# thekingofkings/embedding

Hardware: AMD Instinct MI355X
Metric: SGNS training edges/sec (higher is better)
Workload: dtype f32

## Files before the change

embedding_amd/_native.py:

```python
import ctypes as C
import os

_HERE = os.path.dirname(os.path.abspath(__file__))
LIB_PATH = os.path.join(_HERE, "libdge.so")

DGE_OK, DGE_ERR_ARG, DGE_ERR_RANGE, DGE_ERR_TOPK, DGE_ERR_CAP, DGE_ERR_STATE, DGE_ERR_DEVICE, DGE_ERR_IO = range(8)


class DgeError(RuntimeError):
    def __init__(self, code, msg):
        super().__init__("libdge error %d: %s" % (code, msg))
        self.code = code


class TrainConfig(C.Structure):
    _fields_ = [
        ("dim", C.c_int32), ("window", C.c_int32), ("negative", C.c_int32), ("min_count", C.c_int32),
        ("epochs", C.c_int32), ("workers", C.c_int32), ("alpha", C.c_float), ("min_alpha", C.c_float),
        ("seed", C.c_uint64), ("table_size", C.c_int64), ("n_vertices", C.c_int32), ("update_policy", C.c_int32),
        ("use_hs", C.c_int32), ("reserved", C.c_int32),
    ]


class TrainStats(C.Structure):
# ... 103 lines not shown
    "dge_regions_centroids": (_int, [_vp, _vp, _i64, _P(_i64)]),
    "dge_graph_add_spatial": (_int, [_vp, _vp, _i32, _dbl, _vp, _P(SpatialInfo)]),
    "dge_graph_add_spatial_points": (_int, [_vp, _vp, _vp, _i64, _i32, _dbl, _vp, _P(SpatialInfo)]),
    "dge_trips_parse_texts": (_int, [_int, _vp, _vp, _i32, _P(TripTextOptions), _vp, _vp, _vp, _vp, _i64, _P(_i64), _P(TripTextInfo)]),
    "dge_flows_add_trip_texts": (_int, [_vp, _vp, _vp, _i32, _P(TripTextOptions), _P(TripTextInfo)]),
    "dge_flows_add_trip_files": (_int, [_vp, _vp, _i32, _P(TripTextOptions), _P(TripTextInfo)]),
    "dge_sample_walks": (_int, [_vp, _i64, _i32, _i64, _int, _i64, _vp, _P(_i64)]),
    "dge_sample_walks_device": (_int, [_vp, _i64, _i32, _i64, _int, _i64, _P(_vp), _P(_i64)]),
    "dge_sample_walks_into": (_int, [_vp, _vp, _i64, _i64, _i64, _i64]),
    "dge_walks_from_host": (_int, [_int, _vp, _i64, _i32, _P(_vp)]),
    "dge_names_create": (_int, [_P(_vp)]),
    "dge_names_add": (_int, [_vp, _vp, _i64]),
    "dge_names_count": (_int, [_vp, _P(_i64)]),
    "dge_names_cstrs": (_int, [_vp, _P(_vp)]),
    "dge_names_free": (None, [_vp]),
    "dge_walks_from_seq_text": (_int, [_int, _vp, _i64, _vp, _int, _P(_vp), _P(SeqInfo)]),
    "dge_walks_from_seq_files": (_int, [_int, _vp, _i32, _vp, _int, _P(_vp), _P(SeqInfo)]),
    "dge_walks_to_seq_text": (_int, [_vp, _i64, _i64, _vp, _int, _vp, _i64, _P(_i64), _P(SeqOutInfo)]),
    "dge_walks_write_seq": (_int, [_vp, _i64, _i64, _vp, _int, C.c_char_p, _int, _P(SeqOutInfo)]),
    "dge_walks_to_host": (_int, [_vp, _vp, _i64]),
    "dge_walks_info": (_int, [_vp, _P(_i64), _P(_i32), _P(_vp)]),
    "dge_walks_add_position_prefix": (_int, [_vp, _i32]),
    "dge_walks_free": (None, [_vp]),
    "dge_count_tokens": (_int, [_vp, _i64, _i64, _i32, _vp]),
    "dge_model_create": (_int, [_int, _P(TrainConfig), _vp, _P(_vp)]),
    "dge_model_set_stream": (_int, [_vp, _vp]),
    "dge_model_train": (_int, [_vp, _vp, _i64, _i64, _i64, _i32, _i64, _dbl, _i64]),
    "dge_train_sgns": (_int, [_int, _vp, _i64, _i32, _P(TrainConfig), _P(_vp)]),
    "dge_train_sgns_device": (_int, [_vp, _P(TrainConfig), _P(_vp)]),
    "dge_model_walk_and_train": (_int, [_vp, _vp, _vp, _i64, _i64, _i64, _i64, _i32, _i64, _dbl, _i64]),
    "dge_model_vectors": (_int, [_vp, _P(_vp), _P(_vp), _P(_i64), _P(_i32)]),
    "dge_model_syn1neg": (_int, [_vp, _P(_vp)]),
    "dge_model_syn1": (_int, [_vp, _P(_vp), _P(_i64)]),
    "dge_model_huffman": (_int, [_vp, _P(_vp), _P(_vp), _P(_vp)]),
    "dge_model_counts": (_int, [_vp, _P(_vp)]),
    "dge_model_table": (_int, [_vp, _P(_vp), _P(_i64)]),
    "dge_model_stats": (_int, [_vp, _P(TrainStats)]),
    "dge_model_row_rates": (_int, [_vp, _P(C.c_double), _P(C.c_double), _P(C.c_double), _P(C.c_double)]),
    "dge_model_table_placement": (_int, [_vp, _i32, _vp, _vp, _vp]),
    "dge_model_table_runs": (_int, [_vp, _vp, _vp]),
    "dge_model_tune_placement": (_int, [_vp, _vp, _i64, _i64, _i32, _vp, _vp, _vp]),
    "dge_model_placement_search": (_int, [_vp, _vp, _vp, _vp, _vp]),
    "dge_model_reset_stats": (_int, [_vp]),
    "dge_model_schedule": (_int, [_vp, _P(_i32), _P(_i64), _P(_i32)]),
    "dge_model_kernel": (_int, [_vp, C.c_char_p, _i32]),
    "dge_model_lock_stats": (_int, [_vp, _P(_i64), _P(_i64), _P(_i64)]),
    "dge_model_score_pairs": (_int, [_vp, _vp, _vp, _i64, _vp]),
    "dge_model_eval_links": (_int, [_vp, _vp, _i64, _i64, _i32, C.c_uint64, _P(EvalResult)]),
    "dge_model_eval_sgns": (_int, [_vp, _vp, _i64, _i64, C.c_uint64, _P(EvalResult)]),
    "dge_write_vec": (_int, [_vp, _vp, C.c_char_p, _int]),
    "dge_model_free": (None, [_vp]),
    "dge_model_set_partition": (_int, [_vp, _i32, _i32, _i32]),
    "dge_model_partition_floats": (_int, [_vp, _i32, _P(_i64)]),
    "dge_model_export_partition": (_int, [_vp, _int, _i32, _i32, _vp]),
    "dge_model_import_partition": (_int, [_vp, _int, _i32, _i32, _vp]),
    "dge_model_export_partition_async": (_int, [_vp, _int, _i32, _i32, _vp, _vp]),
    "dge_model_import_partition_async": (_int, [_vp, _int, _i32, _i32, _vp, _vp]),
    "dge_model_stream": (_int, [_vp, _P(_vp)]),
    "dge_host_sync_count": (_int, [_P(_i64)]),
    "dge_model_sync_size": (_int, [_vp, _P(_i64)]),
    "dge_model_snapshot": (_int, [_vp]),
    "dge_model_export_delta": (_int, [_vp, _vp]),
    "dge_model_import_delta": (_int, [_vp, _vp, C.c_float]),
    "dge_comm_unique_id": (_int, [_vp]),
    "dge_comm_create": (_int, [_P(_vp), _vp, _int, _int, _int]),
    "dge_comm_free": (None, [_vp]),
# ... 61 lines not shown
```

embedding_amd/csrc/sgns_io.hip:

```cpp
#include <string.h>

#include <algorithm>
#include <charconv>
#include <string>
#include <thread>
#include <vector>

#include "dge_internal.h"
#include "sgns_kernels.h"
#include "sgns_model.h"
#include "fmt_g9.h"

static int sync_tables_to_host(dge_model* m, bool want_syn0, bool want_syn1, bool want_hs = false) {
    DGE_HIP(hipSetDevice(m->device));
    DGE_HIP(hipStreamSynchronize(m->stream));
    size_t tab = (size_t)m->V * (size_t)m->stride;
    std::vector<float> tmp(tab ? tab : 1);
    for (int which = 0; which < 3; which++) {
        if ((which == 0 && !want_syn0) || (which == 1 && !want_syn1) || (which == 2 && !want_hs)) continue;
        const float* src = which == 0 ? m->d_syn0 : (which == 1 ? m->d_syn1neg : m->d_syn1);
        if (tab) DGE_HIP(hipMemcpy(tmp.data(), src, tab * sizeof(float), hipMemcpyDeviceToHost));
        std::vector<float>& dst = which == 0 ? m->h_syn0 : (which == 1 ? m->h_syn1neg : m->h_syn1);
        const int64_t rows = which == 2 ? std::max<int64_t>(m->V - 1, 0) : m->V;
        dst.resize((size_t)rows * (size_t)m->D + 1);
        for (int64_t r = 0; r < rows; r++) memcpy(dst.data() + r * m->D, tmp.data() + r * m->stride, (size_t)m->D * sizeof(float));
    }
    return DGE_OK;
}

extern "C" int dge_model_vectors(dge_model* m, const float** syn0, const int32_t** vocab_ids, int64_t* V, int32_t* dim) {
    if (!m) DGE_FAIL(DGE_ERR_ARG, "dge_model_vectors: null model");
    int rc = sync_tables_to_host(m, true, false);
    if (rc) return rc;
    if (syn0) *syn0 = m->h_syn0.data();
    if (vocab_ids) *vocab_ids = m->h_vocab_ids.data();
    if (V) *V = m->V;
    if (dim) *dim = m->D;
    return DGE_OK;
}
extern "C" int dge_model_syn1neg(dge_model* m, const float** syn1neg) {
    if (!m || !syn1neg) DGE_FAIL(DGE_ERR_ARG, "dge_model_syn1neg: null argument");
    int rc = sync_tables_to_host(m, false, true);
    if (rc) return rc;
    *syn1neg = m->h_syn1neg.data();
    return DGE_OK;
}
extern "C" int dge_model_syn1(dge_model* m, const float** syn1, int64_t* rows) {
    if (!m || !syn1) DGE_FAIL(DGE_ERR_ARG, "dge_model_syn1: null argument");
    if (!m->d_syn1) DGE_FAIL(DGE_ERR_STATE, "dge_model_syn1: the model was created without use_hs");
    int rc = sync_tables_to_host(m, false, false, true);
    if (rc) return rc;
    *syn1 = m->h_syn1.data();
    if (rows) *rows = std::max<int64_t>(m->V - 1, 0);
    return DGE_OK;
}
extern "C" int dge_model_huffman(dge_model* m, const int64_t** offsets, const int32_t** points, const uint64_t** codes) {
    if (!m) DGE_FAIL(DGE_ERR_ARG, "dge_model_huffman: null model");
    if (!m->d_syn1) DGE_FAIL(DGE_ERR_STATE, "dge_model_huffman: the model was created without use_hs");
    if (offsets) *offsets = m->h_hs_off.data();
    if (points) *points = m->h_hs_points.data();
    if (codes) *codes = m->h_hs_codes.data();
    return DGE_OK;
}
extern "C" int dge_model_counts(dge_model* m, const int64_t** counts) {
    if (!m || !counts) DGE_FAIL(DGE_ERR_ARG, "dge_model_counts: null argument");
    *counts = m->h_counts.data();
    return DGE_OK;
}
__global__ void k_table_unpack(const uint4* __restrict__ ctab, int64_t T, int32_t* __restrict__ table) {
    const int64_t a = (int64_t)blockIdx.x * blockDim.x + threadIdx.x;
    if (a < T) table[a] = neg_table_row(ctab, (uint64_t)a);
}
extern "C" int dge_model_table(dge_model* m, const int32_t** table, int64_t* table_size) {
    if (!m || !table) DGE_FAIL(DGE_ERR_ARG, "dge_model_table: null argument");
    DGE_HIP(hipSetDevice(m->device));
    m->h_table.resize((size_t)m->T);
    dge_tmp<int32_t> flat;
    int rc = flat.alloc((size_t)m->T);
    if (rc) return rc;
    DGE_HIP(hipStreamSynchronize(m->stream));
    hipLaunchKernelGGL(k_table_unpack, dim3(dge_grid_for(m->T, 256)), dim3(256), 0, m->stream, m->d_ctab, m->T, flat.p);
    DGE_HIP(hipStreamSynchronize(m->stream));
    DGE_HIP(hipMemcpy(m->h_table.data(), flat.p, (size_t)m->T * sizeof(int32_t), hipMemcpyDeviceToHost));
    *table = m->h_table.data();
    if (table_size) *table_size = m->T;
    return DGE_OK;
}

extern "C" int dge_write_vec(dge_model* m, const char* const* names, const char* path, int header) {
    if (!m || !path) DGE_FAIL(DGE_ERR_ARG, "dge_write_vec: null argument");
    int rc = sync_tables_to_host(m, true, false);
    if (rc) return rc;
    FILE* f = fopen(path, "w");
    if (!f) DGE_FAIL(DGE_ERR_IO, "dge_write_vec: cannot open %s", path);
    if (header) fprintf(f, "%lld %d\n", (long long)m->V, m->D);
    const int64_t V = m->V; const int D = m->D;
    const unsigned hw = std::thread::hardware_concurrency();
    const int n_thr = (int)std::max<int64_t>(1, std::min<int64_t>(std::min<unsigned>(hw ? hw : 1, 16u), V * (int64_t)D / 65536));
    const int64_t slab = 4096 * (int64_t)n_thr;
    std::vector<std::string> out[2] = {std::vector<std::string>((size_t)n_thr), std::vector<std::string>((size_t)n_thr)};
    bool ok = true;
    std::thread writer;
    int cur = 0;
    for (int64_t r0 = 0; r0 < V; r0 += slab, cur ^= 1) {
        const int64_t r1 = std::min(V, r0 + slab);
        std::vector<std::string>& ob = out[cur];
        auto work = [&, r0, r1](int t) {
            std::string& sbuf = ob[(size_t)t];
            const int64_t a = r0 + (r1 - r0) * t / n_thr, b = r0 + (r1 - r0) * (t + 1) / n_thr;
            size_t cap = 0;
            for (int64_t r = a; r < b; r++) { const int32_t id = m->h_vocab_ids[(size_t)r]; cap += (names && names[id] ? strlen(names[id]) : 12) + (size_t)D * 26 + 2; }
            sbuf.resize(cap);
            char* o = sbuf.data();
            for (int64_t r = a; r < b; r++) {
                const int32_t id = m->h_vocab_ids[(size_t)r];
                if (names && names[id]) { const size_t n = strlen(names[id]); memcpy(o, names[id], n); o += n; } else o = std::to_chars(o, o + 12, id).ptr;
                const float* v = m->h_syn0.data() + r * D;
                for (int j = 0; j < D; j++) {
                    *o++ = ' ';
                    char* e = dge_fmt_g9(v[j], o);
                    o = e ? e : std::to_chars(o, o + 25, (double)v[j], std::chars_format::general, 9).ptr;
                }
                *o++ = '\n';
            }
            sbuf.resize((size_t)(o - sbuf.data()));
        };
        if (n_thr == 1) work(0);
        else {
            std::vector<std::thread> th;
            for (int t = 0; t < n_thr; t++) th.emplace_back(work, t);
            for (auto& x : th) x.join();
        }
        if (writer.joinable()) writer.join();
        if (!ok) break;
        writer = std::thread([&ok, &ob, f, n_thr]() {
            for (int t = 0; t < n_thr && ok; t++) ok = ob[(size_t)t].empty() || fwrite(ob[(size_t)t].data(), 1, ob[(size_t)t].size(), f) == ob[(size_t)t].size();
        });
    }
    if (writer.joinable()) writer.join();
    if (fclose(f) != 0 || !ok) DGE_FAIL(DGE_ERR_IO, "dge_write_vec: write to %s failed", path);
    return DGE_OK;
}

__global__ void k_load_vectors(const int32_t* __restrict__ vocab_ids, int64_t V, int32_t D, int32_t stride, const float* __restrict__ rows, const uint8_t* __restrict__ present,
                               int64_t n_rows, float* __restrict__ syn0, unsigned long long* __restrict__ rows_set) {
    const int64_t i = (int64_t)blockIdx.x * blockDim.x + threadIdx.x;
    if (i >= V * D) return;
    const int64_t r = i / D; const int32_t j = (int32_t)(i - r * D);
    const int64_t id = vocab_ids[r];
    if (id < 0 || id >= n_rows || !present[id]) return;
    syn0[r * stride + j] = rows[id * D + j];
    if (j == 0) atomicAdd(rows_set, 1ull);
}

extern "C" int dge_model_load_vectors(dge_model* m, const dge_vectors* v, int64_t* rows_set) {
    if (!m || !v) DGE_FAIL(DGE_ERR_ARG, "dge_model_load_vectors: null argument");
    if (v->dim != m->D) DGE_FAIL(DGE_ERR_ARG, "dge_model_load_vectors: the vectors have dim %d, the model %d", v->dim, m->D);
    if (v->device != m->device) DGE_FAIL(DGE_ERR_ARG, "dge_model_load_vectors: the vectors are on device %d, the model on %d", v->device, m->device);
    if (m->part_n > 1) DGE_FAIL(DGE_ERR_STATE, "dge_model_load_vectors: a partition is set (n_parts = %d): the tables are in pieces — call dge_model_set_partition(m, 1, 0, 0) first", m->part_n);
    DGE_HIP(hipSetDevice(m->device));
    dge_tmp<unsigned long long> count;
    int rc = count.alloc(1);
    if (rc) return rc;
    DGE_HIP(hipMemsetAsync(count.p, 0, 8, m->stream));
    const int64_t n = m->V * (int64_t)m->D;
    if (n && v->rows) hipLaunchKernelGGL(k_load_vectors, dim3(dge_grid_for(n, 256)), dim3(256), 0, m->stream, m->d_vocab_ids, m->V, m->D, m->stride, v->d, v->d_present, v->rows, m->d_syn0,
                                         count.p);
    DGE_HIP(hipGetLastError());
    unsigned long long set = 0;
    DGE_HIP(hipMemcpyAsync(&set, count.p, 8, hipMemcpyDeviceToHost, m->stream));
    DGE_HIP(hipStreamSynchronize(m->stream));
    if (rows_set) *rows_set = (int64_t)set;
    return DGE_OK;
}
// ... 1 lines not shown
```

embedding_amd/csrc/sgns_model.h:

```cpp
#pragma once
#include <algorithm>
#include <atomic>
#include <string>
#include <vector>

#include "dge_internal.h"
#include "sgns_plan.h"

struct EventPair { hipEvent_t a, b; int kind; };

extern std::atomic<int64_t> g_dge_tuning[DGE_TUNE_COUNT];

struct dge_sorted_work;

struct dge_model {
    int device = 0;
    hipStream_t stream = nullptr;
    bool own_stream = false;
    dge_train_config cfg{};
    int64_t V = 0;
    int32_t D = 0, stride = 0, NV = 0;
    int64_t T = 0;
    ScheduleStats stats;
    BlockHeadMemo block_head_memo;
    int n_cus = 256;
    float *d_syn0 = nullptr, *d_syn1neg = nullptr, *d_snap = nullptr;
    int placed_seen[3] = {0, 0, 0}; double placed_best[3] = {0, 0, 0}, placed_worst[3] = {0, 0, 0};
    float* d_syn1 = nullptr;
    int64_t* d_hs_off = nullptr; int32_t* d_hs_points = nullptr; uint64_t* d_hs_codes = nullptr;
    std::vector<int64_t> h_hs_off; std::vector<int32_t> h_hs_points; std::vector<uint64_t> h_hs_codes;
    std::vector<float> h_syn1;

    int32_t* d_vocab_ids = nullptr;
    int64_t* d_counts = nullptr;
    int32_t* d_remap = nullptr;
    uint4* d_ctab = nullptr; int64_t ctab_blocks = 0;
    double* d_run_base = nullptr; uint32_t* d_run_row = nullptr; uint32_t* d_exc_slot = nullptr; int32_t* d_exc_row = nullptr;
    int32_t n_runs = 0, n_exc = 0;
    float* d_exp = nullptr;
    int64_t cap_rows = 0; int32_t cap_L = 0;
    int32_t* d_sen = nullptr; int64_t* d_len = nullptr; int64_t* d_wb = nullptr;
    void* d_scan_tmp = nullptr; size_t scan_tmp_bytes = 0;
    unsigned long long* d_counters = nullptr;
    int* d_locks = nullptr;
    std::vector<float> h_syn0, h_syn1neg;
    std::vector<int32_t> h_vocab_ids, h_table;
    std::vector<int64_t> h_counts;
    std::vector<EventPair> pending;
    double kernel_ms = 0, walk_ms = 0;
    int64_t launches = 0;
    TrainPlan last_plan; bool has_plan = false;
    int32_t search_runs = 0, search_moved = 0; double search_ms_before = 0, search_ms_after = 0;
    int32_t part_n = 1, part_ctx = 0, part_tgt = 0;
    const int32_t* seen_rows = nullptr; int64_t seen_n = 0; int32_t seen_L = 0; uint64_t seen_gen = 0;
    hipEvent_t ev_peer = nullptr;
    dge_sorted_work* sorted = nullptr;
};

struct TrainParams;
int dge_sorted_train(dge_model* m, const TrainParams& p);
void dge_sorted_release(dge_model* m);

#define DGE_LOCAL __attribute__((visibility("hidden")))
DGE_LOCAL int dge_table_alloc(float** out, size_t floats, int device, hipStream_t st, int* seen, double* rate_best, double* rate_worst);
DGE_LOCAL void dge_table_free(void* p);
DGE_LOCAL int dge_drain_events(dge_model* m);
static inline unsigned dge_grid_for(int64_t n, int block) { return (unsigned)((n + block - 1) / block); }
```

embedding_amd/engine.py:

```python
import ctypes as C
import os

import numpy as np

from ._native import DGE_ERR_CAP, DGE_SLOTS_AS_TRACTS, DGE_SLOTS_EVEN, EvalResult, FlowsInfo, LocateInfo, OdInfo, RegionsInfo, SeqInfo, SeqOutInfo, SpatialInfo, TrainConfig, TrainStats, TripTextInfo, TripTextOptions, VecInfo, check, lib


def _ptr(a):
    return a.ctypes.data_as(C.c_void_p) if a is not None else None


def _dev_ptr(t):
    if t is None:
        return None
    if isinstance(t, int):
        return C.c_void_p(t)
    return C.c_void_p(t.data_ptr())


class DeviceGraph:

    def __init__(self, device=0):
        h = C.c_void_p(0)
        check(lib.dge_graph_create(C.byref(h), int(device)))
# ... 571 lines not shown
    def fit(cls, walks, cfg, device=0):
        h = C.c_void_p(0)
        if isinstance(walks, WalkCorpus):
            check(lib.dge_train_sgns_device(walks._h, C.byref(cfg), C.byref(h)))
            device = walks.device
        else:
            walks = np.ascontiguousarray(walks, np.int32)
            n, L = walks.shape
            check(lib.dge_train_sgns(int(device), _ptr(walks), n, L, C.byref(cfg), C.byref(h)))
        return cls(h, int(device), cfg)

    def close(self):
        if getattr(self, "_h", None):
            lib.dge_model_free(self._h)
            self._h = None

    __del__ = close

    def set_stream(self, stream_ptr):
        check(lib.dge_model_set_stream(self._h, C.c_void_p(int(stream_ptr))))

    def train(self, corpus, row0=0, n_rows=None, walk_index_base=0, epoch=0, words_before=0, words_scale=1.0, total_walks=0):
        if n_rows is None:
            n_rows = corpus.shape[0] - row0
        check(lib.dge_model_train(self._h, corpus._h, int(row0), int(n_rows), int(walk_index_base), int(epoch),
                                  int(words_before), float(words_scale), int(total_walks)))

    def walk_and_train(self, graph, corpus, row0, n_rows, walk_seed, walk_index_base, epoch=0, words_before=0,
                       words_scale=1.0, total_walks=0):
        check(lib.dge_model_walk_and_train(self._h, graph._h, corpus._h, int(row0), int(n_rows), int(walk_seed),
                                           int(walk_index_base), int(epoch), int(words_before), float(words_scale),
                                           int(total_walks)))

    def vectors(self):
        p = C.c_void_p(0); ids = C.c_void_p(0); V = C.c_int64(0); D = C.c_int32(0)
        check(lib.dge_model_vectors(self._h, C.byref(p), C.byref(ids), C.byref(V), C.byref(D)))
        if V.value == 0:
            return np.zeros((0, D.value), np.float32), np.zeros(0, np.int32)
        syn0 = np.ctypeslib.as_array(C.cast(p, C.POINTER(C.c_float)), shape=(V.value * D.value,)).copy().reshape(V.value, D.value)
        vid = np.ctypeslib.as_array(C.cast(ids, C.POINTER(C.c_int32)), shape=(V.value,)).copy()
        return syn0, vid

    def syn1neg(self):
        syn0, _ = self.vectors()
        p = C.c_void_p(0)
        check(lib.dge_model_syn1neg(self._h, C.byref(p)))
        if syn0.size == 0:
            return np.zeros_like(syn0)
        return np.ctypeslib.as_array(C.cast(p, C.POINTER(C.c_float)), shape=(syn0.size,)).copy().reshape(syn0.shape)

    def syn1(self):
        p = C.c_void_p(0); rows = C.c_int64(0)
        check(lib.dge_model_syn1(self._h, C.byref(p), C.byref(rows)))
        n = rows.value * self.cfg.dim
        if n == 0:
            return np.zeros((0, self.cfg.dim), np.float32)
        return np.ctypeslib.as_array(C.cast(p, C.POINTER(C.c_float)), shape=(n,)).copy().reshape(rows.value, self.cfg.dim)

    def huffman(self):
        _, vid = self.vectors()
        V = len(vid)
        po, pp, pc = C.c_void_p(0), C.c_void_p(0), C.c_void_p(0)
        check(lib.dge_model_huffman(self._h, C.byref(po), C.byref(pp), C.byref(pc)))
        if V == 0:
            return np.zeros(1, np.int64), np.zeros(0, np.int32), np.zeros(0, np.uint64)
        off = np.ctypeslib.as_array(C.cast(po, C.POINTER(C.c_int64)), shape=(V + 1,)).copy()
        n = int(off[-1])
        pts = np.ctypeslib.as_array(C.cast(pp, C.POINTER(C.c_int32)), shape=(max(n, 1),)).copy()[:n]
        codes = np.ctypeslib.as_array(C.cast(pc, C.POINTER(C.c_uint64)), shape=(V,)).copy()
        return off, pts, codes

    def counts(self):
        _, vid = self.vectors()
        p = C.c_void_p(0)
        check(lib.dge_model_counts(self._h, C.byref(p)))
        if len(vid) == 0:
            return np.zeros(0, np.int64)
        return np.ctypeslib.as_array(C.cast(p, C.POINTER(C.c_int64)), shape=(len(vid),)).copy()

    def table(self):
        p = C.c_void_p(0); T = C.c_int64(0)
        check(lib.dge_model_table(self._h, C.byref(p), C.byref(T)))
        return np.ctypeslib.as_array(C.cast(p, C.POINTER(C.c_int32)), shape=(T.value,)).copy()

    def row_rates(self):
        v = [C.c_double(0) for _ in range(4)]
        check(lib.dge_model_row_rates(self._h, *[C.byref(x) for x in v])); return tuple(x.value for x in v)

    def table_runs(self):
        n, e = C.c_int32(0), C.c_int32(0)
# ... 95 lines not shown
    def import_partition(self, table, n_parts, part, d_buf):
        check(lib.dge_model_import_partition(self._h, int(table), int(n_parts), int(part), _dev_ptr(d_buf)))

    def export_partition_async(self, table, n_parts, part, d_buf, consumer_stream=0):
        check(lib.dge_model_export_partition_async(self._h, int(table), int(n_parts), int(part), _dev_ptr(d_buf), C.c_void_p(int(consumer_stream))))

    def import_partition_async(self, table, n_parts, part, d_buf, producer_stream=0):
        check(lib.dge_model_import_partition_async(self._h, int(table), int(n_parts), int(part), _dev_ptr(d_buf), C.c_void_p(int(producer_stream))))

    def stream(self):
        p = C.c_void_p(0); check(lib.dge_model_stream(self._h, C.byref(p))); return p.value or 0

    def sync_size(self):
        n = C.c_int64(0); check(lib.dge_model_sync_size(self._h, C.byref(n))); return n.value

    def snapshot(self):
        check(lib.dge_model_snapshot(self._h))

    def export_delta(self, d_buf):
        check(lib.dge_model_export_delta(self._h, _dev_ptr(d_buf)))

    def import_delta(self, d_buf, scale):
        check(lib.dge_model_import_delta(self._h, _dev_ptr(d_buf), float(scale)))


def host_sync_count():
    n = C.c_int64(0); check(lib.dge_host_sync_count(C.byref(n))); return n.value


def build_stamp():
    return dict(kv.split("=") for kv in lib.dge_build_stamp().decode().split())


TUNING_KNOBS = {"hot_rows": 0, "hs_drain": 1, "force_segments": 2, "segment_shift": 3, "sorted_chunk": 4, "sorted_walks": 5, "workers": 6, "static_walks": 7, "hs_cold": 8, "hs_wave": 9, "acc_rows": 10, "acc_drain": 11, "table_runs": 12, "block_syn0_free": 13, "hs_centre": 14, "hs_hot_kb": 15, "allow_unsafe": 16, "watchdog_ms": 17, "hs_copies": 18, "small_rows": 19}


class tuning:

    def __init__(self, **knobs):
        self.knobs = {TUNING_KNOBS[k]: int(v) for k, v in knobs.items()}
        self.before = {}

    def __enter__(self):
        for k, v in self.knobs.items():
            old = C.c_int64(-1)
            check(lib.dge_get_tuning(k, C.byref(old)))
            self.before[k] = old.value
            check(lib.dge_set_tuning(k, v))
        return self

    def __exit__(self, *exc):
        for k in self.knobs:
            check(lib.dge_set_tuning(k, self.before.get(k, -1)))
        return False
```

include/dge.h:

```cpp
#ifndef DGE_H
#define DGE_H
#include <stdint.h>

#ifdef __cplusplus
extern "C" {
#endif

#define DGE_VERSION 106

enum {
    DGE_OK = 0,
    DGE_ERR_ARG = 1,
    DGE_ERR_RANGE = 2,
    DGE_ERR_TOPK = 3,
    DGE_ERR_CAP = 4,
    DGE_ERR_STATE = 5,
    DGE_ERR_DEVICE = 6,
    DGE_ERR_IO = 7
};

typedef struct dge_graph dge_graph;
typedef struct dge_walks dge_walks;
typedef struct dge_model dge_model;

// ... 187 lines not shown
    float   alpha;
    float   min_alpha;
    uint64_t seed;
    int64_t table_size;
    int32_t n_vertices;
    int32_t update_policy;
    int32_t use_hs;
    int32_t reserved;
} dge_train_config;

typedef struct dge_train_stats {
    int64_t pairs;
    int64_t words;
    double  kernel_ms;
    double  walk_kernel_ms;
    int64_t launches;
} dge_train_stats;

int  dge_count_tokens(const dge_walks* w, int64_t row0, int64_t n_rows, int32_t n_vertices, int64_t* d_counts);
int  dge_model_create(int device, const dge_train_config* cfg, const int64_t* d_counts, dge_model** out);
int  dge_model_set_stream(dge_model* m, void* hip_stream);
int  dge_model_train(dge_model* m, const dge_walks* w, int64_t row0, int64_t n_rows, int64_t walk_index_base,
                     int32_t epoch, int64_t words_before, double words_scale, int64_t total_walks_per_epoch);
int  dge_train_sgns(int device, const int32_t* walks , int64_t n_walks, int32_t max_len,
                    const dge_train_config* cfg, dge_model** out);
int  dge_train_sgns_device(const dge_walks* w, const dge_train_config* cfg, dge_model** out);
int  dge_model_walk_and_train(dge_model* m, const dge_graph* g, dge_walks* w, int64_t row0, int64_t n_rows,
                              int64_t walk_seed, int64_t walk_index_base, int32_t epoch, int64_t words_before,
                              double words_scale, int64_t total_walks_per_epoch);
int  dge_model_vectors(dge_model* m, const float** syn0, const int32_t** vocab_ids, int64_t* V, int32_t* dim);
int  dge_model_syn1neg(dge_model* m, const float** syn1neg);
int  dge_model_syn1(dge_model* m, const float** syn1, int64_t* rows);
int  dge_model_huffman(dge_model* m, const int64_t** offsets, const int32_t** points, const uint64_t** codes);
int  dge_model_counts(dge_model* m, const int64_t** counts);
int  dge_model_table(dge_model* m, const int32_t** table, int64_t* table_size);
int  dge_model_stats(const dge_model* m, dge_train_stats* out);
int  dge_model_row_rates(dge_model* m, double* read_gb_per_s, double* rewrite_gb_per_s, double* lock_exchanges_per_s, double* table_lookups_per_s);
int  dge_model_reset_stats(dge_model* m);
int  dge_model_table_placement(const dge_model* m, int32_t table, int32_t* candidates, double* best_gb_per_s, double* worst_gb_per_s);
int  dge_model_table_runs(const dge_model* m, int32_t* n_runs, int32_t* n_exceptions);
int  dge_model_tune_placement(dge_model* m, const dge_walks* w, int64_t row0, int64_t n_rows, int32_t candidates, double* ms_before, double* ms_after,
                              int32_t* arrays_moved);
int  dge_model_placement_search(const dge_model* m, int32_t* runs, double* ms_before, double* ms_after, int32_t* arrays_moved);
int  dge_model_schedule(const dge_model* m, int32_t* update_policy, int64_t* workers, int32_t* hot_rows);
int  dge_model_kernel(const dge_model* m, char* buf, int32_t cap);
int  dge_model_lock_stats(const dge_model* m, int64_t* pairs_put_back, int64_t* rounds_short, int64_t* rounds);
int  dge_host_sync_count(int64_t* n);
typedef struct dge_eval_result {
    int64_t pairs;
    int64_t negatives;
    int64_t skipped;
    double  auc;
    double  loss;
    double  kernel_ms;
} dge_eval_result;

int  dge_model_score_pairs(dge_model* m, const int32_t* d_ctx, const int32_t* d_tgt, int64_t n, float* d_score);

int  dge_model_eval_links(dge_model* m, const dge_walks* w, int64_t row0, int64_t n_rows,
                          int32_t regions_per_slice, uint64_t seed, dge_eval_result* out);

int  dge_model_eval_sgns(dge_model* m, const dge_walks* w, int64_t row0, int64_t n_rows,
                         uint64_t seed, dge_eval_result* out);

int  dge_write_vec(dge_model* m, const char* const* names, const char* path, int header);
void dge_model_free(dge_model* m);
// ... 44 lines not shown
int  dge_vectors_from_vec_text (int device, const char* text, int64_t n_bytes, int header, dge_names* names, int intern, dge_vectors** out, dge_vec_info* info );
int  dge_vectors_from_vec_files(int device, const char* const* paths, int32_t n_paths, int header, dge_names* names, int intern, dge_vectors** out, dge_vec_info* info );
int  dge_vectors_from_host(int device, const float* rows, int64_t n_rows, int32_t dim, const uint8_t* present , dge_vectors** out);
int  dge_vectors_info(const dge_vectors* v, int64_t* rows, int32_t* dim, const float** d_ptr, const uint8_t** d_present);
int  dge_vectors_to_host(const dge_vectors* v, float* out , uint8_t* present , int64_t cap_elems);
void dge_vectors_free(dge_vectors* v);

int  dge_model_load_vectors(dge_model* m, const dge_vectors* v, int64_t* rows_set);

int  dge_knn_cosine_vectors(const dge_vectors* v, int32_t k, int32_t* out_idx, float* out_dist, double* ms_kernel);
int  dge_ndcg_at_k_vectors(const dge_vectors* f, const dge_vectors* gnd, int32_t k, double* ndcg, double* ms_kernels);

enum {
    DGE_TUNE_HOT_ROWS = 0,
    DGE_TUNE_HS_DRAIN = 1,
    DGE_TUNE_FORCE_SEGMENTS = 2,
    DGE_TUNE_SEGMENT_SHIFT = 3,
    DGE_TUNE_SORTED_CHUNK = 4,
    DGE_TUNE_SORTED_WALKS = 5,
    DGE_TUNE_WORKERS = 6,
    DGE_TUNE_STATIC_WALKS = 7,
    DGE_TUNE_HS_COLD = 8,
    DGE_TUNE_HS_WAVE = 9,
    DGE_TUNE_ACC_ROWS = 10,
    DGE_TUNE_ACC_DRAIN = 11,
    DGE_TUNE_TABLE_RUNS = 12,
    DGE_TUNE_BLOCK_SYN0_FREE = 13,
    DGE_TUNE_HS_CENTRE = 14,
    DGE_TUNE_HS_HOT_KB = 15,
    DGE_TUNE_ALLOW_UNSAFE = 16,
    DGE_TUNE_WATCHDOG_MS = 17,
    DGE_TUNE_HS_COPIES = 18,
    DGE_TUNE_SMALL_ROWS = 19,
    DGE_TUNE_COUNT = 20
};
int  dge_set_tuning(int32_t knob, int64_t value);
int  dge_get_tuning(int32_t knob, int64_t* value);

int  dge_selftest_locked_rows(int device, int32_t n_rows, int64_t n_workers, int32_t iters, uint64_t seed,
                              int32_t commit ,
                              int64_t* total_increments, double* max_abs_error);
int  dge_selftest_atomics_wave(int device, int32_t n_rows, int32_t n_acc, int32_t drain, int32_t blocks, int32_t iters, uint64_t seed,
                               int64_t* total_updates, double* max_abs_error);
int  dge_selftest_atomics_wave_block(int device, int32_t n_rows, int32_t n_acc, int32_t drain, int32_t div, int32_t blocks, int32_t iters, uint64_t seed,
                                     int64_t* total_updates, double* max_abs_error);
int  dge_selftest_fmt_g9(int64_t n, uint64_t seed, int64_t* fast_path, int64_t* mismatches);
int  dge_selftest_hot_add(int device, int32_t n_hot, int64_t n_workers, int32_t iters, int32_t drain, uint64_t seed,
                          int64_t* total_additions, double* max_abs_error);
int  dge_selftest_seq_intern(int device, const char* text, int64_t n_bytes, int32_t hash_bits, int64_t initial_slots, int32_t* ids, int64_t cap, int64_t* n_tokens,
                             int64_t* n_names);

#ifdef __cplusplus
}
#endif
#endif
```

Measured before the change: 979.5 million.

## Stream table readback through pinned double-buffered chunks with on-device unpadding

Replaces the full-table pageable device-to-host copy plus host-side row unpadding with a chunked readback. Each chunk is unpadded on the GPU, copied into double-buffered pinned staging, or straight into the destination when it is already pinned, and then copied out on several threads. The vector file writer now formats rows as chunks arrive, overlapping transfer with text formatting. The work targets result extraction, not the training kernels, so the edges/sec metric is unlikely to move, and it adds pinned and device staging memory held by the model.

```diff
diff --git a/embedding_amd/_native.py b/embedding_amd/_native.py
--- a/embedding_amd/_native.py
+++ b/embedding_amd/_native.py
@@ -159,6 +159,7 @@
     "dge_model_vectors": (_int, [_vp, _P(_vp), _P(_vp), _P(_i64), _P(_i32)]),
     "dge_model_syn1neg": (_int, [_vp, _P(_vp)]),
     "dge_model_syn1": (_int, [_vp, _P(_vp), _P(_i64)]),
+    "dge_model_read_table": (_int, [_vp, _i32, _vp, _i64, _P(_i64)]),
     "dge_model_huffman": (_int, [_vp, _P(_vp), _P(_vp), _P(_vp)]),
     "dge_model_counts": (_int, [_vp, _P(_vp)]),
     "dge_model_table": (_int, [_vp, _P(_vp), _P(_i64)]),
diff --git a/embedding_amd/csrc/readback_plan.h b/embedding_amd/csrc/readback_plan.h
--- /dev/null
+++ b/embedding_amd/csrc/readback_plan.h
@@ -0,0 +1,52 @@
+#pragma once
+#include <stdint.h>
+#include <stddef.h>
+
+#define DGE_READBACK_CHUNK_BYTES (64ll << 20)
+
+struct ReadbackPlan {
+    int64_t rows = 0;
+    int32_t width = 0;
+    int32_t stride = 0;
+    int64_t chunk_rows = 1;
+    int64_t n_chunks = 0;
+    bool dense = true;
+    size_t row_bytes() const { return (size_t)width * 4; }
+    size_t chunk_bytes() const { return (size_t)chunk_rows * row_bytes(); }
+    int64_t row0(int64_t k) const { return k * chunk_rows; }
+    int64_t rows_of(int64_t k) const { const int64_t left = rows - k * chunk_rows; return left < chunk_rows ? (left < 0 ? 0 : left) : chunk_rows; }
+    size_t dst_offset(int64_t k) const { return (size_t)row0(k) * row_bytes(); }
+    size_t src_offset(int64_t k) const { return (size_t)row0(k) * (size_t)stride * 4; }
+};
+
+static inline ReadbackPlan readback_plan(int64_t rows, int32_t width, int32_t stride, int64_t chunk_bytes) {
+    ReadbackPlan P;
+    P.rows = rows < 0 ? 0 : rows; P.width = width; P.stride = stride; P.dense = width == stride;
+    if (chunk_bytes <= 0) chunk_bytes = DGE_READBACK_CHUNK_BYTES;
+    const int64_t rb = (int64_t)width * 4;
+    int64_t cr = rb > 0 ? chunk_bytes / rb : 1;
+    if (cr < 1) cr = 1;
+    if (P.rows > 0 && cr > P.rows) cr = P.rows;
+    P.chunk_rows = cr;
+    P.n_chunks = P.rows > 0 && width > 0 ? (P.rows + cr - 1) / cr : 0;
+    return P;
+}
+
+template <class Ops>
+static inline int readback_run(const ReadbackPlan& P, Ops& ops, char* pinned_dst) {
+    int rc = 0;
+    if (pinned_dst) {
+        for (int64_t k = 0; k < P.n_chunks && !rc; k++) rc = ops.issue(k, (int)(k & 1), pinned_dst + P.dst_offset(k));
+        const int rw = P.n_chunks ? ops.wait_all() : 0;
+        return rc ? rc : rw;
+    }
+    for (int64_t k = 0; k < P.n_chunks && k < 2 && !rc; k++) rc = ops.issue(k, (int)k, ops.stage((int)k));
+    for (int64_t k = 0; k < P.n_chunks && !rc; k++) {
+        const int s = (int)(k & 1);
+        if ((rc = ops.wait(s))) break;
+        if ((rc = ops.consume(k, ops.stage(s)))) break;
+        if (k + 2 < P.n_chunks) rc = ops.issue(k + 2, s, ops.stage(s));
+    }
+    if (rc) (void)ops.wait_all();
+    return rc;
+}
diff --git a/embedding_amd/csrc/sgns_io.hip b/embedding_amd/csrc/sgns_io.hip
--- a/embedding_amd/csrc/sgns_io.hip
+++ b/embedding_amd/csrc/sgns_io.hip
@@ -2,6 +2,7 @@
 
 #include <algorithm>
 #include <charconv>
+#include <functional>
 #include <string>
 #include <thread>
 #include <vector>
@@ -9,28 +10,180 @@
 #include "dge_internal.h"
 #include "sgns_kernels.h"
 #include "sgns_model.h"
+#include "readback_plan.h"
 #include "fmt_g9.h"
 
-static int sync_tables_to_host(dge_model* m, bool want_syn0, bool want_syn1, bool want_hs = false) {
+dge_readback_stage::~dge_readback_stage() {
+    for (int s = 0; s < 2; s++) {
+        if (pin[s]) (void)hipHostFree(pin[s]);
+        if (dev[s]) (void)hipFree(dev[s]);
+        if (ev[s]) (void)hipEventDestroy(ev[s]);
+    }
+}
+
+template <int ALIGN>
+__global__ void __launch_bounds__(256) k_unpad_rows(const float* __restrict__ src, int64_t n_rows, int32_t D, int32_t stride, int32_t Q, float* __restrict__ dst) {
+    const int64_t i = (int64_t)blockIdx.x * blockDim.x + threadIdx.x;
+    if (i >= n_rows * Q) return;
+    const int64_t r = i / Q;
+    const int32_t j = (int32_t)(i - r * Q) * 4;
+    const float4 v = *reinterpret_cast<const float4*>(src + r * stride + j);
+    float* o = dst + r * D + j;
+    const int n = min(4, D - j);
+    if (ALIGN == 4) *reinterpret_cast<float4*>(o) = v;
+    else if (ALIGN == 2) {
+        *reinterpret_cast<float2*>(o) = make_float2(v.x, v.y);
+        if (n == 4) *reinterpret_cast<float2*>(o + 2) = make_float2(v.z, v.w);
+    } else {
+        o[0] = v.x;
+        if (n > 1) o[1] = v.y;
+        if (n > 2) o[2] = v.z;
+        if (n > 3) o[3] = v.w;
+    }
+}
+
+struct TableRef { const char* d; int64_t rows; int32_t width, stride; };
+static int table_ref(dge_model* m, int32_t table, TableRef* t, const char* who) {
+    switch (table) {
+        case 0: *t = {(const char*)m->d_syn0, m->V, m->D, m->stride}; return DGE_OK;
+        case 1: *t = {(const char*)m->d_syn1neg, m->V, m->D, m->stride}; return DGE_OK;
+        case 2:
+            if (!m->d_syn1) DGE_FAIL(DGE_ERR_STATE, "%s: the model was created without use_hs", who);
+            *t = {(const char*)m->d_syn1, std::max<int64_t>(m->V - 1, 0), m->D, m->stride}; return DGE_OK;
+        case 3: *t = {(const char*)m->d_vocab_ids, m->V, 1, 1}; return DGE_OK;
+    }
+    DGE_FAIL(DGE_ERR_ARG, "%s: unknown table %d", who, table);
+}
+
+static bool host_pinned(const void* p, size_t bytes) {
+    const char* ends[2] = {(const char*)p, (const char*)p + (bytes ? bytes - 1 : 0)};
+    for (const char* q : ends) {
+        hipPointerAttribute_t a{};
+        if (hipPointerGetAttributes(&a, q) != hipSuccess) { (void)hipGetLastError(); return false; }
+        if (a.type != hipMemoryTypeHost) return false;
+    }
+    return true;
+}
+
+static bool stage_ensure(dge_model* m, size_t bytes, bool want_pin, bool want_dev) {
+    dge_readback_stage& st = m->readback;
+    for (int s = 0; s < 2; s++)
+        if (!st.ev[s] && hipEventCreateWithFlags(&st.ev[s], hipEventDisableTiming) != hipSuccess) { st.ev[s] = nullptr; (void)hipGetLastError(); return false; }
+    if (want_pin && st.pin_bytes < bytes) {
+        for (int s = 0; s < 2; s++) { if (st.pin[s]) (void)hipHostFree(st.pin[s]); st.pin[s] = nullptr; }
+        st.pin_bytes = 0;
+        for (int s = 0; s < 2; s++)
+            if (hipHostMalloc(&st.pin[s], bytes, hipHostMallocDefault) != hipSuccess) { st.pin[s] = nullptr; (void)hipGetLastError(); return false; }
+        st.pin_bytes = bytes;
+    }
+    if (want_dev && st.dev_bytes < bytes) {
+        for (int s = 0; s < 2; s++) { if (st.dev[s]) (void)hipFree(st.dev[s]); st.dev[s] = nullptr; }
+        st.dev_bytes = 0;
+        for (int s = 0; s < 2; s++)
+            if (hipMalloc((void**)&st.dev[s], bytes) != hipSuccess) { st.dev[s] = nullptr; (void)hipGetLastError(); return false; }
+        st.dev_bytes = bytes;
+    }
+    return true;
+}
+
+static void copy_out(char* dst, const char* src, size_t bytes) {
+    const unsigned hw = std::thread::hardware_concurrency();
+    const size_t n_thr = std::min<size_t>(std::min<size_t>(hw ? hw : 1, 4), bytes >> 22);
+    if (n_thr <= 1) { memcpy(dst, src, bytes); return; }
+    std::vector<std::thread> th;
+    for (size_t t = 0; t < n_thr; t++) {
+        const size_t a = bytes * t / n_thr / 64 * 64, b = t + 1 == n_thr ? bytes : bytes * (t + 1) / n_thr / 64 * 64;
+        th.emplace_back([=]() { memcpy(dst + a, src + a, b - a); });
+    }
+    for (auto& x : th) x.join();
+}
+
+struct ReadbackOps {
+    dge_model* m; const ReadbackPlan& P; const TableRef& t; bool direct;
+    const std::function<int(int64_t, const char*)>& consume_fn;
+    int issue(int64_t k, int slot, char* to) {
+        dge_readback_stage& st = m->readback;
+        const int64_t n = P.rows_of(k);
+        const void* from = t.d + P.src_offset(k);
+        if (!P.dense) {
+            const int32_t D = P.width, Q = (D + 3) / 4;
+            const float* src = (const float*)from;
+            const dim3 g(dge_grid_for(n * Q, 256)), b(256);
+            if (D % 4 == 0) hipLaunchKernelGGL(k_unpad_rows<4>, g, b, 0, m->stream, src, n, D, P.stride, Q, st.dev[slot]);
+            else if (D % 2 == 0) hipLaunchKernelGGL(k_unpad_rows<2>, g, b, 0, m->stream, src, n, D, P.stride, Q, st.dev[slot]);
+            else hipLaunchKernelGGL(k_unpad_rows<1>, g, b, 0, m->stream, src, n, D, P.stride, Q, st.dev[slot]);
+            DGE_HIP(hipGetLastError());
+            from = st.dev[slot];
+        }
+        DGE_HIP(hipMemcpyAsync(to, from, (size_t)n * P.row_bytes(), hipMemcpyDeviceToHost, m->stream));
+        if (!direct) DGE_HIP(hipEventRecord(st.ev[slot], m->stream));
+        return DGE_OK;
+    }
+    int wait(int slot) { DGE_HIP(hipEventSynchronize(m->readback.ev[slot])); return DGE_OK; }
+    int wait_all() { DGE_HIP(hipStreamSynchronize(m->stream)); return DGE_OK; }
+    char* stage(int slot) { return (char*)m->readback.pin[slot]; }
+    int consume(int64_t k, const char* from) { return consume_fn(k, from); }
+};
+
+static int readback_pageable(dge_model* m, const TableRef& t, char* dst) {
+    DGE_HIP(hipStreamSynchronize(m->stream));
+    const size_t words = (size_t)t.rows * (size_t)t.stride;
+    if (!words) return DGE_OK;
+    if (t.width == t.stride) { DGE_HIP(hipMemcpy(dst, t.d, words * 4, hipMemcpyDeviceToHost)); return DGE_OK; }
+    std::vector<uint32_t> tmp(words);
+    DGE_HIP(hipMemcpy(tmp.data(), t.d, words * 4, hipMemcpyDeviceToHost));
+    for (int64_t r = 0; r < t.rows; r++) memcpy(dst + (size_t)r * t.width * 4, tmp.data() + (size_t)r * t.stride, (size_t)t.width * 4);
+    return DGE_OK;
+}
+
+static int readback_staged(dge_model* m, const TableRef& t, char* dst, const std::function<int(const char*, int64_t, int64_t)>* rows_fn, bool* staged) {
+    *staged = false;
+    if (g_dge_tuning[DGE_TUNE_READBACK_PAGEABLE] > 0 || (t.width != t.stride && t.stride % 4 != 0)) return DGE_OK;
+    const ReadbackPlan P = readback_plan(t.rows, t.width, t.stride, g_dge_tuning[DGE_TUNE_READBACK_CHUNK]);
+    const bool direct = !rows_fn && host_pinned(dst, (size_t)t.rows * P.row_bytes());
+    if (P.n_chunks && !stage_ensure(m, P.chunk_bytes(), !direct, !P.dense)) return DGE_OK;
+    *staged = true;
+    const std::function<int(int64_t, const char*)> consume = [&](int64_t k, const char* from) -> int {
+        if (rows_fn) return (*rows_fn)(from, P.row0(k), P.rows_of(k));
+        copy_out(dst + P.dst_offset(k), from, (size_t)P.rows_of(k) * P.row_bytes());
+        return DGE_OK;
+    };
+    ReadbackOps ops{m, P, t, direct, consume};
+    return readback_run(P, ops, direct ? dst : nullptr);
+}
+
+static int read_table(dge_model* m, const TableRef& t, char* dst) {
     DGE_HIP(hipSetDevice(m->device));
-    DGE_HIP(hipStreamSynchronize(m->stream));
-    size_t tab = (size_t)m->V * (size_t)m->stride;
-    std::vector<float> tmp(tab ? tab : 1);
-    for (int which = 0; which < 3; which++) {
-        if ((which == 0 && !want_syn0) || (which == 1 && !want_syn1) || (which == 2 && !want_hs)) continue;
-        const float* src = which == 0 ? m->d_syn0 : (which == 1 ? m->d_syn1neg : m->d_syn1);
-        if (tab) DGE_HIP(hipMemcpy(tmp.data(), src, tab * sizeof(float), hipMemcpyDeviceToHost));
-        std::vector<float>& dst = which == 0 ? m->h_syn0 : (which == 1 ? m->h_syn1neg : m->h_syn1);
-        const int64_t rows = which == 2 ? std::max<int64_t>(m->V - 1, 0) : m->V;
-        dst.resize((size_t)rows * (size_t)m->D + 1);
-        for (int64_t r = 0; r < rows; r++) memcpy(dst.data() + r * m->D, tmp.data() + r * m->stride, (size_t)m->D * sizeof(float));
-    }
-    return DGE_OK;
+    bool staged = false;
+    const int rc = readback_staged(m, t, dst, nullptr, &staged);
+    if (rc || staged) return rc;
+    return readback_pageable(m, t, dst);
+}
+
+extern "C" int dge_model_read_table(dge_model* m, int32_t table, void* dst, int64_t dst_bytes, int64_t* rows) {
+    if (!m) DGE_FAIL(DGE_ERR_ARG, "dge_model_read_table: null model");
+    TableRef t;
+    int rc = table_ref(m, table, &t, "dge_model_read_table");
+    if (rc) return rc;
+    if (rows) *rows = t.rows;
+    if (!dst) return DGE_OK;
+    const int64_t need = t.rows * (int64_t)t.width * 4;
+    if (dst_bytes < need) DGE_FAIL(DGE_ERR_ARG, "dge_model_read_table: table %d is %lld bytes, dst holds %lld", table, (long long)need, (long long)dst_bytes);
+    return read_table(m, t, (char*)dst);
+}
+
+static int sync_table_to_host(dge_model* m, int32_t table, const char* who) {
+    TableRef t;
+    int rc = table_ref(m, table, &t, who);
+    if (rc) return rc;
+    std::vector<float>& dst = table == 0 ? m->h_syn0 : (table == 1 ? m->h_syn1neg : m->h_syn1);
+    dst.resize((size_t)t.rows * (size_t)t.width + 1);
+    return read_table(m, t, (char*)dst.data());
 }
 
 extern "C" int dge_model_vectors(dge_model* m, const float** syn0, const int32_t** vocab_ids, int64_t* V, int32_t* dim) {
     if (!m) DGE_FAIL(DGE_ERR_ARG, "dge_model_vectors: null model");
-    int rc = sync_tables_to_host(m, true, false);
+    int rc = sync_table_to_host(m, 0, "dge_model_vectors");
     if (rc) return rc;
     if (syn0) *syn0 = m->h_syn0.data();
     if (vocab_ids) *vocab_ids = m->h_vocab_ids.data();
@@ -40,15 +193,14 @@
 }
 extern "C" int dge_model_syn1neg(dge_model* m, const float** syn1neg) {
     if (!m || !syn1neg) DGE_FAIL(DGE_ERR_ARG, "dge_model_syn1neg: null argument");
-    int rc = sync_tables_to_host(m, false, true);
+    int rc = sync_table_to_host(m, 1, "dge_model_syn1neg");
     if (rc) return rc;
     *syn1neg = m->h_syn1neg.data();
     return DGE_OK;
 }
 extern "C" int dge_model_syn1(dge_model* m, const float** syn1, int64_t* rows) {
     if (!m || !syn1) DGE_FAIL(DGE_ERR_ARG, "dge_model_syn1: null argument");
-    if (!m->d_syn1) DGE_FAIL(DGE_ERR_STATE, "dge_model_syn1: the model was created without use_hs");
-    int rc = sync_tables_to_host(m, false, false, true);
+    int rc = sync_table_to_host(m, 2, "dge_model_syn1");
     if (rc) return rc;
     *syn1 = m->h_syn1.data();
     if (rows) *rows = std::max<int64_t>(m->V - 1, 0);
@@ -87,59 +239,85 @@
     return DGE_OK;
 }
 
+struct VecWriter {
+    dge_model* m; const char* const* names; FILE* f; int D; int n_thr; int64_t slab;
+    std::vector<std::string> out[2];
+    bool ok = true;
+    std::thread writer;
+    int cur = 0;
+    VecWriter(dge_model* m_, const char* const* names_, FILE* f_) : m(m_), names(names_), f(f_), D(m_->D) {
+        const unsigned hw = std::thread::hardware_concurrency();
+        n_thr = (int)std::max<int64_t>(1, std::min<int64_t>(std::min<unsigned>(hw ? hw : 1, 16u), m->V * (int64_t)D / 65536));
+        slab = 4096 * (int64_t)n_thr;
+        out[0].resize((size_t)n_thr); out[1].resize((size_t)n_thr);
+    }
+    bool rows(const float* v, int64_t r0, int64_t r1) {
+        for (int64_t s0 = r0; s0 < r1 && ok; s0 += slab, cur ^= 1) {
+            const int64_t s1 = std::min(r1, s0 + slab);
+            std::vector<std::string>& ob = out[cur];
+            auto work = [&, s0, s1](int t) {
+                std::string& sbuf = ob[(size_t)t];
+                const int64_t a = s0 + (s1 - s0) * t / n_thr, b = s0 + (s1 - s0) * (t + 1) / n_thr;
+                size_t cap = 0;
+                for (int64_t r = a; r < b; r++) { const int32_t id = m->h_vocab_ids[(size_t)r]; cap += (names && names[id] ? strlen(names[id]) : 12) + (size_t)D * 26 + 2; }
+                sbuf.resize(cap);
+                char* o = sbuf.data();
+                for (int64_t r = a; r < b; r++) {
+                    const int32_t id = m->h_vocab_ids[(size_t)r];
+                    if (names && names[id]) { const size_t n = strlen(names[id]); memcpy(o, names[id], n); o += n; } else o = std::to_chars(o, o + 12, id).ptr;
+                    const float* x = v + (r - r0) * D;
+                    for (int j = 0; j < D; j++) {
+                        *o++ = ' ';
+                        char* e = dge_fmt_g9(x[j], o);
+                        o = e ? e : std::to_chars(o, o + 25, (double)x[j], std::chars_format::general, 9).ptr;
+                    }
+                    *o++ = '\n';
+                }
+                sbuf.resize((size_t)(o - sbuf.data()));
+            };
+            if (n_thr == 1) work(0);
+            else {
+                std::vector<std::thread> th;
+                for (int t = 0; t < n_thr; t++) th.emplace_back(work, t);
+                for (auto& x : th) x.join();
+            }
+            if (writer.joinable()) writer.join();
+            if (!ok) break;
+            writer = std::thread([this, &ob]() {
+                for (int t = 0; t < n_thr && ok; t++) ok = ob[(size_t)t].empty() || fwrite(ob[(size_t)t].data(), 1, ob[(size_t)t].size(), f) == ob[(size_t)t].size();
+            });
+        }
+        return ok;
+    }
+    bool finish() { if (writer.joinable()) writer.join(); return ok; }
+    ~VecWriter() { if (writer.joinable()) writer.join(); }
+};
+
 extern "C" int dge_write_vec(dge_model* m, const char* const* names, const char* path, int header) {
     if (!m || !path) DGE_FAIL(DGE_ERR_ARG, "dge_write_vec: null argument");
-    int rc = sync_tables_to_host(m, true, false);
-    if (rc) return rc;
+    DGE_HIP(hipSetDevice(m->device));
+    TableRef t;
+    int rc = table_ref(m, 0, &t, "dge_write_vec");
+    if (rc) return rc;
+    const bool want_staged = g_dge_tuning[DGE_TUNE_READBACK_PAGEABLE] <= 0;
+    if (!want_staged && (rc = sync_table_to_host(m, 0, "dge_write_vec"))) return rc;
     FILE* f = fopen(path, "w");
     if (!f) DGE_FAIL(DGE_ERR_IO, "dge_write_vec: cannot open %s", path);
     if (header) fprintf(f, "%lld %d\n", (long long)m->V, m->D);
-    const int64_t V = m->V; const int D = m->D;
-    const unsigned hw = std::thread::hardware_concurrency();
-    const int n_thr = (int)std::max<int64_t>(1, std::min<int64_t>(std::min<unsigned>(hw ? hw : 1, 16u), V * (int64_t)D / 65536));
-    const int64_t slab = 4096 * (int64_t)n_thr;
-    std::vector<std::string> out[2] = {std::vector<std::string>((size_t)n_thr), std::vector<std::string>((size_t)n_thr)};
-    bool ok = true;
-    std::thread writer;
-    int cur = 0;
-    for (int64_t r0 = 0; r0 < V; r0 += slab, cur ^= 1) {
-        const int64_t r1 = std::min(V, r0 + slab);
-        std::vector<std::string>& ob = out[cur];
-        auto work = [&, r0, r1](int t) {
-            std::string& sbuf = ob[(size_t)t];
-            const int64_t a = r0 + (r1 - r0) * t / n_thr, b = r0 + (r1 - r0) * (t + 1) / n_thr;
-            size_t cap = 0;
-            for (int64_t r = a; r < b; r++) { const int32_t id = m->h_vocab_ids[(size_t)r]; cap += (names && names[id] ? strlen(names[id]) : 12) + (size_t)D * 26 + 2; }
-            sbuf.resize(cap);
-            char* o = sbuf.data();
-            for (int64_t r = a; r < b; r++) {
-                const int32_t id = m->h_vocab_ids[(size_t)r];
-                if (names && names[id]) { const size_t n = strlen(names[id]); memcpy(o, names[id], n); o += n; } else o = std::to_chars(o, o + 12, id).ptr;
-                const float* v = m->h_syn0.data() + r * D;
-                for (int j = 0; j < D; j++) {
-                    *o++ = ' ';
-                    char* e = dge_fmt_g9(v[j], o);
-                    o = e ? e : std::to_chars(o, o + 25, (double)v[j], std::chars_format::general, 9).ptr;
-                }
-                *o++ = '\n';
-            }
-            sbuf.resize((size_t)(o - sbuf.data()));
-        };
-        if (n_thr == 1) work(0);
-        else {
-            std::vector<std::thread> th;
-            for (int t = 0; t < n_thr; t++) th.emplace_back(work, t);
-            for (auto& x : th) x.join();
+    bool ok;
+    {
+        VecWriter w(m, names, f);
+        bool staged = false;
+        if (want_staged) {
+            const std::function<int(const char*, int64_t, int64_t)> fn = [&w](const char* v, int64_t r0, int64_t n) { return w.rows((const float*)v, r0, r0 + n) ? DGE_OK : DGE_ERR_IO; };
+            rc = readback_staged(m, t, nullptr, &fn, &staged);
+            if (!rc && !staged) rc = sync_table_to_host(m, 0, "dge_write_vec");
         }
-        if (writer.joinable()) writer.join();
-        if (!ok) break;
-        writer = std::thread([&ok, &ob, f, n_thr]() {
-            for (int t = 0; t < n_thr && ok; t++) ok = ob[(size_t)t].empty() || fwrite(ob[(size_t)t].data(), 1, ob[(size_t)t].size(), f) == ob[(size_t)t].size();
-        });
-    }
-    if (writer.joinable()) writer.join();
-    if (fclose(f) != 0 || !ok) DGE_FAIL(DGE_ERR_IO, "dge_write_vec: write to %s failed", path);
-    return DGE_OK;
+        if (!rc && !staged) w.rows(m->h_syn0.data(), 0, m->V);
+        ok = w.finish();
+    }
+    if (fclose(f) != 0 || (!ok && (!rc || rc == DGE_ERR_IO))) DGE_FAIL(DGE_ERR_IO, "dge_write_vec: write to %s failed", path);
+    return rc;
 }
 
 __global__ void k_load_vectors(const int32_t* __restrict__ vocab_ids, int64_t V, int32_t D, int32_t stride, const float* __restrict__ rows, const uint8_t* __restrict__ present,
diff --git a/embedding_amd/csrc/sgns_model.h b/embedding_amd/csrc/sgns_model.h
--- a/embedding_amd/csrc/sgns_model.h
+++ b/embedding_amd/csrc/sgns_model.h
@@ -12,6 +12,16 @@
 extern std::atomic<int64_t> g_dge_tuning[DGE_TUNE_COUNT];
 
 struct dge_sorted_work;
+
+struct dge_readback_stage {
+    void* pin[2] = {nullptr, nullptr}; size_t pin_bytes = 0;
+    float* dev[2] = {nullptr, nullptr}; size_t dev_bytes = 0;
+    hipEvent_t ev[2] = {nullptr, nullptr};
+    dge_readback_stage() = default;
+    dge_readback_stage(const dge_readback_stage&) = delete;
+    dge_readback_stage& operator=(const dge_readback_stage&) = delete;
+    ~dge_readback_stage();
+};
 
 struct dge_model {
     int device = 0;
@@ -46,6 +56,7 @@
     std::vector<float> h_syn0, h_syn1neg;
     std::vector<int32_t> h_vocab_ids, h_table;
     std::vector<int64_t> h_counts;
+    dge_readback_stage readback;
     std::vector<EventPair> pending;
     double kernel_ms = 0, walk_ms = 0;
     int64_t launches = 0;
diff --git a/embedding_amd/engine.py b/embedding_amd/engine.py
--- a/embedding_amd/engine.py
+++ b/embedding_amd/engine.py
@@ -627,30 +627,33 @@
                                            int(walk_index_base), int(epoch), int(words_before), float(words_scale),
                                            int(total_walks)))
 
+    def read_table(self, table, out=None):
+        rows = C.c_int64(0)
+        check(lib.dge_model_read_table(self._h, int(table), None, 0, C.byref(rows)))
+        shape, dt = ((rows.value,), np.int32) if table == 3 else ((rows.value, self.cfg.dim), np.float32)
+        if out is None:
+            out = np.empty(shape, dt)
+        if isinstance(out, np.ndarray):
+            if out.dtype != dt or not out.flags["C_CONTIGUOUS"] or not out.flags["WRITEABLE"]:
+                raise ValueError("read_table: out must be a writeable C-contiguous %s array" % np.dtype(dt).name)
+            ptr, nbytes = out.ctypes.data, out.nbytes
+        else:
+            if out.device.type != "cpu" or not out.is_contiguous() or out.element_size() != 4:
+                raise ValueError("read_table: out must be a contiguous CPU tensor of 4-byte elements")
+            ptr, nbytes = out.data_ptr(), out.numel() * 4
+        if nbytes != int(np.prod(shape)) * 4:
+            raise ValueError("read_table: out holds %d bytes, the table %d" % (nbytes, int(np.prod(shape)) * 4))
+        check(lib.dge_model_read_table(self._h, int(table), C.c_void_p(ptr), nbytes, None))
+        return out
+
     def vectors(self):
-        p = C.c_void_p(0); ids = C.c_void_p(0); V = C.c_int64(0); D = C.c_int32(0)
-        check(lib.dge_model_vectors(self._h, C.byref(p), C.byref(ids), C.byref(V), C.byref(D)))
-        if V.value == 0:
-            return np.zeros((0, D.value), np.float32), np.zeros(0, np.int32)
-        syn0 = np.ctypeslib.as_array(C.cast(p, C.POINTER(C.c_float)), shape=(V.value * D.value,)).copy().reshape(V.value, D.value)
-        vid = np.ctypeslib.as_array(C.cast(ids, C.POINTER(C.c_int32)), shape=(V.value,)).copy()
-        return syn0, vid
+        return self.read_table(0), self.read_table(3)
 
     def syn1neg(self):
-        syn0, _ = self.vectors()
-        p = C.c_void_p(0)
-        check(lib.dge_model_syn1neg(self._h, C.byref(p)))
-        if syn0.size == 0:
-            return np.zeros_like(syn0)
-        return np.ctypeslib.as_array(C.cast(p, C.POINTER(C.c_float)), shape=(syn0.size,)).copy().reshape(syn0.shape)
+        return self.read_table(1)
 
     def syn1(self):
-        p = C.c_void_p(0); rows = C.c_int64(0)
-        check(lib.dge_model_syn1(self._h, C.byref(p), C.byref(rows)))
-        n = rows.value * self.cfg.dim
-        if n == 0:
-            return np.zeros((0, self.cfg.dim), np.float32)
-        return np.ctypeslib.as_array(C.cast(p, C.POINTER(C.c_float)), shape=(n,)).copy().reshape(rows.value, self.cfg.dim)
+        return self.read_table(2)
 
     def huffman(self):
         _, vid = self.vectors()
@@ -812,7 +815,7 @@
     return dict(kv.split("=") for kv in lib.dge_build_stamp().decode().split())
 
 
-TUNING_KNOBS = {"hot_rows": 0, "hs_drain": 1, "force_segments": 2, "segment_shift": 3, "sorted_chunk": 4, "sorted_walks": 5, "workers": 6, "static_walks": 7, "hs_cold": 8, "hs_wave": 9, "acc_rows": 10, "acc_drain": 11, "table_runs": 12, "block_syn0_free": 13, "hs_centre": 14, "hs_hot_kb": 15, "allow_unsafe": 16, "watchdog_ms": 17, "hs_copies": 18, "small_rows": 19}
+TUNING_KNOBS = {"hot_rows": 0, "hs_drain": 1, "force_segments": 2, "segment_shift": 3, "sorted_chunk": 4, "sorted_walks": 5, "workers": 6, "static_walks": 7, "hs_cold": 8, "hs_wave": 9, "acc_rows": 10, "acc_drain": 11, "table_runs": 12, "block_syn0_free": 13, "hs_centre": 14, "hs_hot_kb": 15, "allow_unsafe": 16, "watchdog_ms": 17, "hs_copies": 18, "small_rows": 19, "readback_chunk": 20, "readback_pageable": 21}
 
 
 class tuning:
diff --git a/include/dge.h b/include/dge.h
--- a/include/dge.h
+++ b/include/dge.h
@@ -243,6 +243,7 @@
 int  dge_model_syn1neg(dge_model* m, const float** syn1neg);
 int  dge_model_syn1(dge_model* m, const float** syn1, int64_t* rows);
 int  dge_model_huffman(dge_model* m, const int64_t** offsets, const int32_t** points, const uint64_t** codes);
+int  dge_model_read_table(dge_model* m, int32_t table, void* dst, int64_t dst_bytes, int64_t* rows);
 int  dge_model_counts(dge_model* m, const int64_t** counts);
 int  dge_model_table(dge_model* m, const int32_t** table, int64_t* table_size);
 int  dge_model_stats(const dge_model* m, dge_train_stats* out);
@@ -353,7 +354,9 @@
     DGE_TUNE_WATCHDOG_MS = 17,
     DGE_TUNE_HS_COPIES = 18,
     DGE_TUNE_SMALL_ROWS = 19,
-    DGE_TUNE_COUNT = 20
+    DGE_TUNE_READBACK_CHUNK = 20,
+    DGE_TUNE_READBACK_PAGEABLE = 21,
+    DGE_TUNE_COUNT = 22
 };
 int  dge_set_tuning(int32_t knob, int64_t value);
 int  dge_get_tuning(int32_t knob, int64_t* value);
```

New measurement: 979.4 million. About the same (-0.0%).
